# thomeou/SALSA

Measured on AMD Instinct MI355X. Metric: SALSA feat-extract audio-s/s, higher is better.
Workload: dtype f64 (STFT, noise-floor tracker, eigen-solve cold list) + packed f32 (covariance and eigen-solve of the certified frames); 1 GPU; Full SALSA FOA (eigenvector path): batch 32x60-s 4-ch 24 kHz clips per GPU, feature-extract only, n_fft 512 hop 300 fmax_doa 9000 cond 5 tracking on; clips_per_gpu=32, feature=salsa, format=foa, clip_groups=default

## Files before the change

salsa_amd/csrc/salsa_internal.h:

```cpp
#pragma once
#include <hip/hip_runtime.h>
#include <stdio.h>

#include "../../include/salsa_hip.h"
#include "salsa_math.h"

#define SALSA_LOCAL __attribute__((visibility("hidden")))

extern "C" SALSA_LOCAL void salsa_set_last_error_(const char *msg);

namespace salsa_impl {

static inline int fail(int code, const char *fmt, const char *a = "", long b = 0)
{
    char msg[512];
    snprintf(msg, sizeof(msg), fmt, a, b);
    salsa_set_last_error_(msg);
    return code;
}

static inline int hip_fail(const char *expr, hipError_t e)
{
    char msg[512];
    snprintf(msg, sizeof(msg), "%s failed: %s", expr, hipGetErrorString(e));
// ... 7 lines not shown
        if (e_ != hipSuccess) return salsa_impl::hip_fail(#expr, e_);                             \
    } while (0)

struct KParams {
    int B;
    int N;
    int T;
    int hop;
    int lower, upper, nd;
    int cutoff;
    int F;
    int OC;
    int ident;
    int spec_lo, spec_hi;
    int flex;
    int compress;
    int layout;
    int feature;
    int format;
    int tracking;
    int n_hop;
    int pair_sel;
    int nch;
    double cond;
    double inv_cond;
    double delta;
    double snr_ratio;
    const float *sc_mean;
    const float *sc_std;
    unsigned long long *stats;
    int force_f64;
    unsigned *doubt32;
    unsigned *doubt_flag;
};

constexpr int FEATURE_LOGSPEC_ONLY = 3;

constexpr int TR_CH = 64;
constexpr int TR_BINS = 32;
#ifndef K3_FT_N
#define K3_FT_N 8
#endif
constexpr int K3_FT = K3_FT_N;
#ifndef K3_NT_N
#define K3_NT_N 128
#endif
constexpr int K3_NT = K3_NT_N;
#ifndef SALSA_PK
#define SALSA_PK 1
#endif
#define SALSA_PK_COND_MIN 2.0

__device__ __forceinline__ int swz(int e) { return e ^ ((e >> 3) & 7); }

__device__ __forceinline__ void wave_lds_fence()
{
    __builtin_amdgcn_fence(__ATOMIC_RELEASE, "wavefront");
    __builtin_amdgcn_wave_barrier();
    __builtin_amdgcn_fence(__ATOMIC_ACQUIRE, "wavefront");
}

__device__ __forceinline__ float power32(const float2 x)
{
    const float t = x.x * x.x;
    return __builtin_fmaf(x.y, x.y, t);
}
// ... 69 lines not shown
```

salsa_amd/csrc/salsa_kernels.hip:

```cpp
#include "build_guard.h"
#include "salsa_internal.h"
#include <type_traits>

using salsa::cplx;
using namespace salsa_impl;

namespace {

template <int N> struct fft_cfg {
    static constexpr int NSUB = (N == 1024) ? 2 : 1;
    static constexpr int NS = N / NSUB;
    static constexpr int R = (NS == 512) ? 8 : 4;
    static constexpr int NP = (NS == 512) ? 2 : 3;
};

template <typename V> __device__ __forceinline__ V ld_off_c(const V *base, unsigned byte_off, int const_bytes) { return *(const V *)((const char *)base + byte_off + const_bytes); }
#ifndef K1_SPILL_NT
#define K1_SPILL_NT 1
#endif
typedef float salsa_f4v __attribute__((ext_vector_type(4)));
#ifndef TR_NT_LD
#define TR_NT_LD 0
#endif
#ifndef K3_GATHER_NT
// ... 449 lines not shown
        const double re = x[i].x, im = x[i].y;
        p[i] = re * re + im * im;
    }
#pragma unroll
    for (int i = 0; i < COUNT; i++) {
        if (first + i < TR_CH)
            dst[(first + i) * BINS + col] = raw ? sqrt(p[i + 2]) : sqrt(div3_exact(((0.0 + p[i + 2]) + p[i + 1]) + p[i]));
    }
}

#ifndef TR_IDLE4
#define TR_IDLE4 1
#endif
#ifndef TR_MASK_HISTORY
#define TR_MASK_HISTORY 1
#endif
#ifndef TR_CHUNK_CLAMP_SKIP
#define TR_CHUNK_CLAMP_SKIP 0
#endif
#ifndef TR_LAZY_CLAMP
#define TR_LAZY_CLAMP 0
#endif
extern "C" __device__ int salsa_writelane_i32(int value, int lane, int old) __asm("llvm.amdgcn.writelane.i32");
#ifndef TR_WIDE
#define TR_WIDE 0
#endif
constexpr int TR_WG_BINS = TR_WIDE ? 64 : TR_BINS;
static unsigned tracker_grid(const KParams &kp) { return (unsigned)(kp.B * ((kp.nd + TR_WG_BINS - 1) / TR_WG_BINS)); }

__global__ __launch_bounds__(64 * TR_WAVES) void tracker_kernel(const KParams kp, const float4 *__restrict__ Xs,
                                                                unsigned *__restrict__ valid32)
{
    if (kp.doubt_flag && blockIdx.x == 0 && threadIdx.x == 0) *kp.doubt_flag = 0u;
    constexpr int BINS = TR_WG_BINS, FS = 64 / BINS;
    constexpr bool IDLE4 = TR_WAVES > 4 && TR_IDLE4;
    constexpr int NPROD = IDLE4 ? TR_WAVES - 2 : TR_WAVES - 1;
    constexpr int PER_ALL = (TR_CH + TR_WAVES * FS - 1) / (TR_WAVES * FS);
    constexpr int PER_PROD = (TR_CH + NPROD * FS - 1) / (NPROD * FS);
    __shared__ double ring[2][TR_CH * BINS];
    const int ng32 = (kp.nd + BINS - 1) / BINS;
    const int b = blockIdx.x / ng32, g = blockIdx.x % ng32;
    const int w = __builtin_amdgcn_readfirstlane(threadIdx.x >> 6), lane = threadIdx.x & 63;
    const int col = lane % BINS, fsub = lane / BINS;
    const int bin = g * BINS + col;
    const bool active = bin < kp.nd;
    const int Tn = kp.T;
    const int stride = (kp.nch / 2) * kp.nd;
    const float4 *x0 = Xs + (long)b * Tn * stride + (active ? bin : 0);
    const int nchunks = (Tn + TR_CH - 1) / TR_CH;
    const bool raw = kp.flex != 0;
    {
        float2 x[PER_ALL + 2];
        const int first = (w * FS + fsub) * PER_ALL;
        tracker_load<PER_ALL>(kp, x0, stride, 0, first, active, x);
        tracker_mag<PER_ALL, BINS>(x, first, ring[0], col, raw);
    }
    float2 xa[PER_PROD + 2], xb[PER_PROD + 2];
    const bool producer = w > 0 && !(IDLE4 && w == 4);
    const int pidx = (IDLE4 && w > 4) ? w - 2 : w - 1;
    const int pfirst = (pidx * FS + fsub) * PER_PROD;
    if (producer && nchunks > 1) tracker_load<PER_PROD>(kp, x0, stride, TR_CH, pfirst, active, xa);
    __syncthreads();
    double fl = 0.0;
    int cd = 3;
    const double snr = kp.snr_ratio;
    const int n32 = (kp.nd + TR_BINS - 1) / TR_BINS;
// ... 119 lines not shown
#ifndef TR_PROBE_NO_PRODUCE
            if (w != 0 && producer) produce(c + 1, xb, xa);
#endif
        }
        chunk_barrier();
    }
}

#ifndef K3_GROUP
#define K3_GROUP 2
#endif
constexpr int K3_OW = K3_NT + 8;
#ifndef K3_XCD_CHUNK
#define K3_XCD_CHUNK 16
#endif

#ifndef K3_STAGE_LDS
#define K3_STAGE_LDS 0
#endif
#ifndef K3_OUT_NT
#define K3_OUT_NT 1
#endif
#ifndef K3_PK_WAVES
#define K3_PK_WAVES 4
#endif
template <bool FEAT, int NHOP, bool FAST = false, bool PK = false>
__global__ __launch_bounds__(K3_NT, PK ? K3_PK_WAVES : 1) void cov_eig_kernel(const KParams kp, const float4 *__restrict__ Xs,
                                                      const unsigned *__restrict__ valid32,
                                                      float *__restrict__ out_feat, double *__restrict__ out_eig,
                                                      unsigned char *__restrict__ gate)
{
    constexpr int G = NHOP >= 0 ? K3_GROUP : 1;
    constexpr bool PAIRED = G > 1;
    static_assert(K3_FT % G == 0 && G <= 4 && K3_FT / G <= 16, "work-list entry layout");
    __shared__ unsigned short list[K3_FT * K3_NT];
    __shared__ unsigned short slow[FAST ? K3_FT * K3_NT : 1];
    __shared__ int count, nslow;
    __shared__ __attribute__((aligned(16))) unsigned rowoff[NHOP >= 0 ? K3_FT + 2 * NHOP + 2 : 2];
    __shared__ __attribute__((aligned(16))) float otile[FEAT ? 3 * K3_FT * K3_OW : 4];
#if K3_STAGE_LDS
    __shared__ __attribute__((aligned(16))) float4 stage[PK ? (K3_FT + 6) * 2 * K3_NT : 1];
#endif
    const int tid = threadIdx.x;
    const int Tn = kp.T;
    int tile = blockIdx.x, b = blockIdx.y;
    if (K3_XCD_CHUNK > 0) {
        const unsigned ntile = gridDim.x, total = ntile * gridDim.y, lin = blockIdx.x + ntile * blockIdx.y;
        constexpr unsigned span = 8u * (K3_XCD_CHUNK > 0 ? K3_XCD_CHUNK : 1);
        if (lin < total / span * span) {
            const unsigned xcd = lin & 7u, j = lin >> 3;
            const unsigned tl = ((j / (span / 8)) * 8u + xcd) * (span / 8) + j % (span / 8);
            b = (int)(tl / ntile);
            tile = (int)(tl - (unsigned)b * ntile);
        }
    }
    const int t0 = tile * K3_FT;
    const int nft = Tn - t0 < K3_FT ? Tn - t0 : K3_FT;
    const int bin0 = blockIdx.z * K3_NT;
    const int nbc = kp.nd - bin0 < K3_NT ? kp.nd - bin0 : K3_NT;
    if (tid == 0) count = 0, nslow = 0;
    if (kp.doubt32 && tid < K3_FT * (K3_NT / 32)) {
        const int ft = tid % K3_FT, g32 = bin0 / 32 + tid / K3_FT, n32 = (kp.nd + TR_BINS - 1) / TR_BINS;
        if (ft < nft && g32 < n32) kp.doubt32[((long)b * n32 + g32) * Tn + t0 + ft] = 0u;
    }
    if (NHOP >= 0 && tid < K3_FT + 2 * NHOP) {
        int tt = t0 - NHOP + tid;
        while (tt < 0) tt += Tn;
        while (tt >= Tn) tt -= Tn;
        rowoff[tid] = (unsigned)tt * (16u * 2u * (unsigned)kp.nd);
    }
    if (FEAT) {
        for (int i = tid; i < 3 * K3_FT * K3_OW / 4; i += K3_NT) ((float4 *)otile)[i] = make_float4(0.f, 0.f, 0.f, 0.f);
    }
    __syncthreads();
    float *of = FEAT ? out_feat + ((long)b * kp.OC + 4) * Tn * kp.F : nullptr;
    double *oe = FEAT ? nullptr : out_eig + (long)b * 3 * kp.nd * Tn;
    unsigned char *og = (!FEAT && gate) ? gate + (long)b * kp.nd * Tn : nullptr;
    auto emit = [&](int t, int bin, const double *e, unsigned char g) {
        if (FEAT) {
#pragma unroll
            for (int i = 0; i < 3; i++) otile[(i * K3_FT + (t - t0)) * K3_OW + (bin - bin0)] = (float)e[i];
        } else {
#pragma unroll
            for (int i = 0; i < 3; i++) oe[((long)i * kp.nd + bin) * Tn + t] = e[i];
            if (og) og[(long)bin * Tn + t] = g;
        }
    };
    const double zero3[3] = {0.0, 0.0, 0.0};
    {
        const int bl = tid;
        const bool in = bl < nbc;
        const int ng32 = (kp.nd + TR_BINS - 1) / TR_BINS;
        const int bin = bin0 + bl;
        const int lane = tid & 63;
        const int grp = __builtin_amdgcn_readfirstlane(bin >> 6);
        const unsigned long long inmask = __ballot(in);
// ... 22 lines not shown
        int base = 0;
        if (lane == 0 && total) base = atomicAdd(&count, total);
        base = __builtin_amdgcn_readfirstlane(base);
#pragma unroll
        for (int ft = 0; ft < K3_FT; ft += G) {
            const unsigned long long wd = any_of(ft);
            if (in) {
                unsigned v = 0;
#pragma unroll
                for (int j = 0; j < G; j++) v |= ((unsigned)(words[ft + j] >> lane) & 1u) << j;
                if (v) list[base + __popcll(wd & ((1ull << lane) - 1))] = (unsigned short)((v << 12) | ((ft / G) << 8) | bl);
#pragma unroll
                for (int j = 0; j < G; j++)
                    if (!FEAT && ft + j < nft && !((v >> j) & 1)) emit(t0 + ft + j, bin, zero3, 0);
            }
            base += __popcll(wd);
        }
    }
    const int seg = (FEAT && blockIdx.z == gridDim.z - 1) ? (kp.F - bin0 < K3_OW ? kp.F - bin0 : K3_OW) : nbc;
    if (FEAT && blockIdx.z == gridDim.z - 1 && kp.F - bin0 > K3_OW) {
        const int first = bin0 + K3_OW, tail = kp.F - first;
        for (int i = tid; i < nft * tail; i += K3_NT) {
            const int ft = i / tail, f = first + (i - ft * tail);
#pragma unroll
            for (int c = 0; c < 3; c++) st_off(of, 4u * (unsigned)((c * Tn + t0 + ft) * kp.F + f), 0.f);
        }
    }
    __syncthreads();
    const int n = count;
    const int stride = 2 * kp.nd;
    const int nhop = NHOP >= 0 ? NHOP : kp.n_hop;
    const float4 *xclip = Xs + (long)b * Tn * stride;
    const bool ungated = !kp.tracking && !kp.flex;
    auto solve_emit = [&](const salsa::herm4<double> &R, int t, int bin, auto path) {
        constexpr int PATH = decltype(path)::value;
        const bool foa = kp.format == SALSA_FORMAT_FOA;
        const salsa::eig_result<double> er = salsa::herm4_gate_eigvec<PATH>(R, kp.cond, kp.inv_cond, ungated, !foa);
        if (PATH == 1 && er.fallback) {
            slow[atomicAdd(&nslow, 1)] = (unsigned short)(((t - t0) << 8) | (bin - bin0));
            return;
        }
        if (er.doubt && kp.doubt32 && !ungated) {
            atomicOr(&kp.doubt32[((long)b * ((kp.nd + TR_BINS - 1) / TR_BINS) + (bin >> 5)) * Tn + t], 1u << (bin & 31));
            atomicOr(kp.doubt_flag, 1u);
        }
        double e[3] = {0.0, 0.0, 0.0};
        unsigned char g = er.rank1 ? 2 : 1;
        if (er.rank1 || ungated) {
            const int k = bin + kp.lower;
            const double den = kp.flex ? (double)((float)(k == 0 ? 1 : k) * (float)kp.delta) : kp.delta * (double)k;
            if (PATH != 2 && er.col0) {
                if (foa) salsa::normalise_foa_col0(er.u, e);
                else salsa::normalise_mic_col0(er.u, den, e);
            } else if (PATH != 1) {
                if (foa) salsa::normalise_foa(er.u, e, ungated);
                else salsa::normalise_mic(er.u, den, e);
            }
            g = 2;
        } else if (FEAT && kp.flex && !kp.tracking) {
            e[0] = __builtin_nan("");
        }
        emit(t, bin, e, g);
    };
    using hot_path = std::integral_constant<int, FAST ? 1 : 2>;
    using cold_path = std::integral_constant<int, 2>;
    if constexpr (PK) {
        static_assert(!PK || (G == 2 && FEAT && FAST && NHOP >= 0), "the packed solve takes the two frames of a pair");
        constexpr int NW = 2 * NHOP + 2;
        const unsigned half = 16u * (unsigned)kp.nd;
#if K3_STAGE_LDS
        if (n > 0) {
            for (int i = tid; i < (K3_FT + 6) * 2 * K3_NT; i += K3_NT) {
// ... 26 lines not shown
            auto chans = [&](int k, salsa::pk2f *v) {
                v[0] = salsa::pk2f{xa[k].x, xa[k].y};
                v[1] = salsa::pk2f{xa[k].z, xa[k].w};
                v[2] = salsa::pk2f{xc[k].x, xc[k].y};
                v[3] = salsa::pk2f{xc[k].z, xc[k].w};
            };
            salsa::cov4pk Cc = {}, C0, C1;
            salsa::pk2f v[4];
#pragma unroll
            for (int k = 1; k <= 2 * NHOP; k++) {
                chans(k, v);
                salsa::cov4pk_rank1(Cc, Cc, v);
            }
            chans(0, v);
            salsa::cov4pk_rank1(C0, Cc, v);
            chans(2 * NHOP + 1, v);
            salsa::cov4pk_rank1(C1, Cc, v);
            const int live = (i >> 12) & 3;
            int odd;
            const salsa::herm4<salsa::pk2f> A = salsa::herm4_pk_from_windows(C0, C1, odd);
            salsa::pk2f e[3];
            salsa::pk_eig r;
            if (kp.format == SALSA_FORMAT_FOA) {
                r = salsa::herm4_gate_eigvec_pk<false>(A, (float)kp.cond, (float)kp.inv_cond, live & ~odd);
                if (r.pass) salsa::normalise_foa_pk(r, e);
            } else {
                r = salsa::herm4_gate_eigvec_pk<true>(A, (float)kp.cond, (float)kp.inv_cond, live & ~odd);
                if (r.pass) salsa::normalise_mic_pk(r, (float)(kp.delta * (double)(bin0 + bl + kp.lower)), e);
            }
            r.unsure |= odd & live;
#pragma unroll
            for (int j = 0; j < 2; j++) {
                if ((r.unsure >> j) & 1)
                    slow[atomicAdd(&nslow, 1)] = (unsigned short)(((ft + j) << 8) | bl);
                else if ((r.pass >> j) & 1) {
#pragma unroll
                    for (int q = 0; q < 3; q++) otile[(q * K3_FT + ft + j) * K3_OW + bl] = e[q][j];
                }
            }
        }
    }
    for (int s = tid; !PK && s < n; s += K3_NT) {
        const int i = list[s];
        const int t = t0 + G * ((i >> 8) & 15);
        const int bin = bin0 + (i & 255);
        const float4 *xb = xclip + bin;
        const unsigned row = 16u * (unsigned)stride, boff = 16u * (unsigned)bin, half = 16u * (unsigned)kp.nd;
        if (PAIRED) {
            constexpr int NW = NHOP >= 0 ? 2 * NHOP + G : G;
            float4 xa[NW], xc[NW];
            const unsigned *ro = rowoff + (t - t0);
#pragma unroll
            for (int k = 0; k < NW; k++) {
                const unsigned r = ro[k];
                xa[k] = ld_off(xclip, r + boff);
                xc[k] = ld_off(xclip, r + boff + half);
            }
            auto frame = [&](int k, salsa::herm4<double> &A) {
                const cplx<double> x[4] = {{(double)xa[k].x, (double)xa[k].y}, {(double)xa[k].z, (double)xa[k].w},
                                           {(double)xc[k].x, (double)xc[k].y}, {(double)xc[k].z, (double)xc[k].w}};
                salsa::herm4_rank1_add(A, x);
            };
            salsa::herm4<double> Rc = {};
#pragma unroll
            for (int k = G - 1; k <= 2 * NHOP; k++) frame(k, Rc);
#pragma unroll
            for (int j = 0; j < G; j++) {
                if ((i >> (12 + j)) & 1) {
                    salsa::herm4<double> R = Rc;
#pragma unroll
                    for (int k = j; k < G - 1; k++) frame(k, R);
#pragma unroll
                    for (int k = 2 * NHOP + 1; k <= 2 * NHOP + j; k++) frame(k, R);
                    solve_emit(R, t + j, bin, hot_path{});
                }
            }
        } else {
            salsa::herm4<double> R = {};
            for (int k = -nhop; k <= nhop; k++) {
                int tt = t + k;
                while (tt < 0) tt += Tn;
                while (tt >= Tn) tt -= Tn;
                const float4 a = xb[tt * stride], c = xb[tt * stride + kp.nd];
                const cplx<double> x[4] = {{(double)a.x, (double)a.y}, {(double)a.z, (double)a.w},
                                           {(double)c.x, (double)c.y}, {(double)c.z, (double)c.w}};
                salsa::herm4_rank1_add(R, x);
            }
            solve_emit(R, t, bin, hot_path{});
        }
    }
    if (FAST) {
        __syncthreads();
        const int ns = nslow;
        if (kp.stats && tid == 0) {
            int live = 0;
            for (int s = 0; s < n; s++) live += __popc((list[s] >> 12) & 15);
            atomicAdd(&kp.stats[0], (unsigned long long)n);
            atomicAdd(&kp.stats[1], (unsigned long long)live);
            atomicAdd(&kp.stats[2], (unsigned long long)ns);
            atomicAdd(&kp.stats[3], 1ull);
        }
        for (int s = tid; s < ns; s += K3_NT) {
            const int i = slow[s];
            const int t = t0 + (i >> 8), bin = bin0 + (i & 255);
            const float4 *xb = xclip + bin;
            salsa::herm4<double> R = {};
            for (int k = -nhop; k <= nhop; k++) {
                int tt = t + k;
                while (tt < 0) tt += Tn;
                while (tt >= Tn) tt -= Tn;
                const float4 a = xb[tt * stride], c = xb[tt * stride + kp.nd];
                const cplx<double> x[4] = {{(double)a.x, (double)a.y}, {(double)a.z, (double)a.w},
                                           {(double)c.x, (double)c.y}, {(double)c.z, (double)c.w}};
                salsa::herm4_rank1_add(R, x);
            }
            solve_emit(R, t, bin, cold_path{});
        }
    }
    if (FEAT) {
        __syncthreads();
        const bool vec = !(kp.F & 3) && !(seg & 3) && !(bin0 & 3);
        if (vec) {
            const int q = seg >> 2;
            for (int i = tid; i < 3 * nft * q; i += K3_NT) {
                const int row = i / q, col = i - row * q, c = row / nft, ft = row - c * nft;
                float4 *dst = (float4 *)(of + ((long)(c * Tn + t0 + ft) * kp.F + bin0 + 4 * col));
                const float4 val = *(const float4 *)(otile + (c * K3_FT + ft) * K3_OW + 4 * col);
                if (K3_OUT_NT) st_off_nt(dst, 0u, val);
                else *dst = val;
            }
        } else {
            for (int i = tid; i < 3 * nft * seg; i += K3_NT) {
                const int row = i / seg, col = i - row * seg, c = row / nft, ft = row - c * nft;
                of[(long)(c * Tn + t0 + ft) * kp.F + bin0 + col] = otile[(c * K3_FT + ft) * K3_OW + col];
            }
        }
    }
}

template <bool FEAT>
__global__ __launch_bounds__(256) void gate_doubt_kernel(const KParams kp, const float4 *__restrict__ Xs, float *__restrict__ out_feat,
                                                         double *__restrict__ out_eig, unsigned char *__restrict__ gate)
{
    if (*(const volatile unsigned *)kp.doubt_flag == 0u) return;
    const int Tn = kp.T, n32 = (kp.nd + TR_BINS - 1) / TR_BINS, stride = 2 * kp.nd;
    const long nwords = (long)kp.B * n32 * Tn;
    const bool foa = kp.format == SALSA_FORMAT_FOA;
    for (long wi = (long)blockIdx.x * blockDim.x + threadIdx.x; wi < nwords; wi += (long)gridDim.x * blockDim.x) {
        unsigned word = kp.doubt32[wi];
        if (!word) continue;
        const int t = (int)(wi % Tn), g32 = (int)((wi / Tn) % n32), b = (int)(wi / ((long)Tn * n32));
        while (word) {
            const int j = __ffs((int)word) - 1;
            word &= word - 1u;
            const int bin = 32 * g32 + j;
            const float4 *xb = Xs + (long)b * Tn * stride + bin;
            salsa::herm4<double> R = {};
            for (int k = -kp.n_hop; k <= kp.n_hop; k++) {
                int tt = t + k;
                while (tt < 0) tt += Tn;
                while (tt >= Tn) tt -= Tn;
                const float4 a = xb[tt * stride], c = xb[tt * stride + kp.nd];
                const cplx<double> x[4] = {{(double)a.x, (double)a.y}, {(double)a.z, (double)a.w},
                                           {(double)c.x, (double)c.y}, {(double)c.z, (double)c.w}};
                salsa::herm4_rank1_add(R, x);
            }
            const bool rank1 = salsa::herm4_rank1_by_jacobi(R, kp.cond);
            double e[3] = {0.0, 0.0, 0.0};
            if (rank1) {
                const salsa::eig_result<double> er = salsa::herm4_gate_eigvec<2>(R, kp.cond, kp.inv_cond, true, !foa);
                const int k = bin + kp.lower;
                const double den = kp.flex ? (double)((float)(k == 0 ? 1 : k) * (float)kp.delta) : kp.delta * (double)k;
                if (foa) salsa::normalise_foa(er.u, e, false);
                else salsa::normalise_mic(er.u, den, e);
            } else if (FEAT && kp.flex && !kp.tracking) {
                e[0] = __builtin_nan("");
            }
            if (FEAT) {
#pragma unroll
                for (int i = 0; i < 3; i++) out_feat[(((long)b * kp.OC + 4 + i) * Tn + t) * kp.F + bin] = (float)e[i];
            } else {
#pragma unroll
                for (int i = 0; i < 3; i++) out_eig[(((long)b * 3 + i) * kp.nd + bin) * Tn + t] = e[i];
                if (gate) gate[((long)b * kp.nd + bin) * Tn + t] = rank1 ? 2 : 1;
            }
        }
    }
}

__global__ __launch_bounds__(256) void flex_allpass_kernel(const KParams kp, float *__restrict__ out)
{
    const int bin = blockIdx.x * 256 + threadIdx.x;
    if (bin >= kp.nd) return;
    float *of = out + ((long)blockIdx.y * kp.OC + kp.nch) * kp.T * kp.F + bin;
    bool dead = false;
    for (int t = 0; t < kp.T; t++) {
        const float v = of[t * kp.F];
        dead = dead || (v != v);
        if (dead) {
            for (int c = 0; c < kp.nch - 1; c++) of[(c * kp.T + t) * kp.F] = 0.f;
        }
    }
}

}

namespace salsa_impl {

void launch_tracker(const KParams &kp, hipStream_t s, const float4 *Xs, unsigned *valid32)
{
    hipLaunchKernelGGL(tracker_kernel, dim3(tracker_grid(kp)), dim3(64 * TR_WAVES), 0, s, kp, Xs, valid32);
}

template <bool FEAT>
static void launch_gate_doubt(const KParams &kp, hipStream_t s, const float4 *Xs, float *out_feat, double *out_eig, unsigned char *gate)
{
    if (!kp.doubt32) return;
    const long nwords = (long)kp.B * ((kp.nd + TR_BINS - 1) / TR_BINS) * kp.T;
    const unsigned blocks = (unsigned)(nwords < 256L * 64 ? (nwords + 255) / 256 : 64);
    hipLaunchKernelGGL(gate_doubt_kernel<FEAT>, dim3(blocks ? blocks : 1u), dim3(256), 0, s, kp, Xs, out_feat, out_eig, gate);
}

template <bool FEAT>
void launch_cov_eig(const KParams &kp, dim3 grid, hipStream_t s, const float4 *Xs, const unsigned *valid,
                    float *out_feat, double *out_eig, unsigned char *gate)
{
    const bool gated = kp.tracking || kp.flex;
    if (kp.doubt32 && !kp.tracking) (void)hipMemsetAsync(kp.doubt_flag, 0, sizeof(unsigned), s);
    if (FEAT && SALSA_PK && K3_GROUP == 2 && kp.n_hop == 3 && gated && SALSA_COL0 && !kp.flex && kp.cond >= SALSA_PK_COND_MIN && kp.cond < 1e6 && !kp.force_f64)
        hipLaunchKernelGGL((cov_eig_kernel<FEAT, 3, true, FEAT && K3_GROUP == 2>), grid, dim3(K3_NT), 0, s, kp, Xs, valid, out_feat, out_eig, gate);
    else if (kp.n_hop == 3 && gated && SALSA_COL0)
        hipLaunchKernelGGL((cov_eig_kernel<FEAT, 3, true>), grid, dim3(K3_NT), 0, s, kp, Xs, valid, out_feat, out_eig, gate);
    else if (kp.n_hop == 3)
        hipLaunchKernelGGL((cov_eig_kernel<FEAT, 3>), grid, dim3(K3_NT), 0, s, kp, Xs, valid, out_feat, out_eig, gate);
    else
        hipLaunchKernelGGL((cov_eig_kernel<FEAT, -1>), grid, dim3(K3_NT), 0, s, kp, Xs, valid, out_feat, out_eig, gate);
    launch_gate_doubt<FEAT>(kp, s, Xs, out_feat, out_eig, gate);
}

template void launch_cov_eig<true>(const KParams &, dim3, hipStream_t, const float4 *, const unsigned *, float *, double *, unsigned char *);
template void launch_cov_eig<false>(const KParams &, dim3, hipStream_t, const float4 *, const unsigned *, float *, double *, unsigned char *);

void launch_flex_allpass(const KParams &kp, hipStream_t s, float *out)
{
    hipLaunchKernelGGL(flex_allpass_kernel, dim3((unsigned)((kp.nd + 255) / 256), (unsigned)kp.B), dim3(256), 0, s, kp, out);
}

int launch_stft(salsa_plan *pl, const KParams &kp, const double *win, const float *d_audio, float *d_out, float4 *Xs, hipStream_t s)
{
    const bool lite = kp.feature == SALSA_FEATURE_LITE || kp.feature == SALSA_FEATURE_IPD;
    const bool single = !lite && kp.pair_sel >= 0;
    constexpr int NF_FULL = k1_cfg<false>::NF, NF_LITE = k1_cfg<true>::NF, NF_PAIR = 2 * k1_cfg<false>::NF;
    const int fpb = 4 * (lite ? NF_LITE : single ? NF_PAIR : NF_FULL);
    const unsigned nblk = (unsigned)((kp.T + fpb - 1) / fpb);
    dim3 grid(nblk, (unsigned)kp.B);
    const bool one_window = pl->d_window == pl->d_window_doa;
    const bool std_layout = K1_STD && one_window && pl->p.n_fft == 512 && !lite && !single && kp.feature == SALSA_FEATURE_SALSA && kp.compress &&
                            kp.spec_lo == 1 && kp.spec_hi == 193 && kp.ident == 192 && kp.F == 200 && kp.nch == 4 &&
                            kp.layout == SALSA_LAYOUT_PLANAR && kp.pair_sel < 0;
    const bool lite_std = K1_LITE_STD && one_window && pl->p.n_fft == 512 && lite && kp.nch == 4 && kp.layout == SALSA_LAYOUT_PLANAR && !kp.sc_mean &&
                          kp.cutoff <= 256 && kp.pair_sel < 0;
    if (lite_std) {
        hipLaunchKernelGGL((stft_kernel<512, double, true, NF_LITE, 2, false, true>), grid, dim3(256), 0, s, kp, d_audio, win, pl->d_tw, d_out, Xs);
    } else if (std_layout) {
        constexpr size_t SCT_BYTES = 2 * 4 * 256 * sizeof(float);
        if (kp.sc_mean) hipLaunchKernelGGL((stft_kernel<512, double, false, NF_FULL, 2, true, true>), grid, dim3(256), SCT_BYTES, s, kp, d_audio, win, pl->d_tw, d_out, Xs);
        else hipLaunchKernelGGL((stft_kernel<512, double, false, NF_FULL, 2, false, true>), grid, dim3(256), 0, s, kp, d_audio, win, pl->d_tw, d_out, Xs);
    } else if (pl->p.n_fft == 1024) {
        if (!lite) return fail(SALSA_ENFFT, "n_fft 1024 is a SALSA-Lite / SALSA-IPD size%s");
        hipLaunchKernelGGL((stft_kernel<1024, double, true, NF_LITE>), grid, dim3(256), 0, s, kp, d_audio, win, pl->d_tw, d_out, Xs);
// ... 49 lines not shown
```

salsa_amd/csrc/salsa_plan.hip:

```cpp
#include "build_guard.h"
#include "salsa_internal.h"
#include <string.h>

using salsa::cplx;
using namespace salsa_impl;

namespace {

thread_local char g_err[512] = "";

}

namespace salsa_impl {

KParams make_kparams(const salsa_plan *pl, int batch, int64_t n_samples)
{
    KParams kp;
    memset(&kp, 0, sizeof(kp));
    kp.B = batch;
    kp.N = (int)n_samples;
    kp.T = (int)(1 + n_samples / pl->p.hop_len);
    kp.hop = pl->p.hop_len;
    kp.lower = pl->lower;
    kp.upper = pl->upper;
// ... 184 lines not shown

int salsa_plan_destroy(salsa_plan *pl)
{
    if (!pl) return SALSA_OK;
    if (pl->d_window) (void)hipFree(pl->d_window);
    if (pl->d_tw) (void)hipFree(pl->d_tw);
    for (int i = 0; i < SALSA_MAX_KERNELS; i++) {
        if (pl->ev0[i]) (void)hipEventDestroy(pl->ev0[i]);
        if (pl->ev1[i]) (void)hipEventDestroy(pl->ev1[i]);
    }
    for (int i = 0; i <= SALSA_MAX_GROUPS; i++) {
        if (pl->streams[i]) (void)hipStreamDestroy(pl->streams[i]);
        if (pl->ev_join[i]) (void)hipEventDestroy(pl->ev_join[i]);
        if (i < SALSA_MAX_GROUPS && pl->ev_stft[i]) (void)hipEventDestroy(pl->ev_stft[i]);
        if (i < SALSA_MAX_GROUPS && pl->ev_stft2[i]) (void)hipEventDestroy(pl->ev_stft2[i]);
    }
    if (pl->gexec) (void)hipGraphExecDestroy(pl->gexec);
    if (pl->cap_stream) (void)hipStreamDestroy(pl->cap_stream);
    if (pl->ev_fork) (void)hipEventDestroy(pl->ev_fork);
    delete pl;
    return SALSA_OK;
}

int salsa_output_shape(const salsa_plan *pl, int64_t n_samples, int *C, int64_t *T, int *F)
{
    if (!pl || n_samples < 0) return fail(SALSA_EINVAL, "salsa_output_shape: bad argument%s");
    if (C) *C = 7;
    if (T) *T = 1 + n_samples / pl->p.hop_len;
    if (F) *F = pl->F;
    return SALSA_OK;
}

static size_t mask_bytes(int batch, size_t T, int nd) { return align256((size_t)batch * ((T + 63) / 64) * ((nd + 63) / 64) * 64 * 8); }

size_t salsa_workspace_bytes(const salsa_plan *pl, int batch, int64_t n_samples)
{
    if (!pl || batch <= 0 || n_samples <= 0 || pl->p.feature_type != SALSA_FEATURE_SALSA) return 0;
    const size_t T = 1 + n_samples / pl->p.hop_len;
    return align256((size_t)batch * T * 4 * pl->nd * sizeof(float2)) + 2 * mask_bytes(batch, T, pl->nd) + align256(sizeof(unsigned) * (size_t)batch) + 256;
}

size_t salsa_eigvec_workspace_bytes(const salsa_plan *pl, int batch, int n_bins, int64_t n_frames)
{
    if (!pl || batch <= 0 || n_bins <= 0 || n_frames <= 0) return 0;
    return align256((size_t)batch * n_frames * 4 * n_bins * sizeof(float2)) + 2 * mask_bytes(batch, (size_t)n_frames, n_bins) + align256(sizeof(unsigned) * (size_t)batch) + 256;
}

static int mark_begin(salsa_plan *pl, hipStream_t s, const char *name)
{
    if (!pl->timing || pl->n_kernels >= SALSA_MAX_KERNELS) return -1;
    const int i = pl->n_kernels++;
    pl->names[i] = name;
    if (!pl->ev0[i]) (void)hipEventCreate(&pl->ev0[i]);
    if (!pl->ev1[i]) (void)hipEventCreate(&pl->ev1[i]);
    (void)hipEventRecord(pl->ev0[i], s);
    return i;
}
static void mark_end(salsa_plan *pl, hipStream_t s, int i)
{
    if (i >= 0) (void)hipEventRecord(pl->ev1[i], s);
}

int salsa_extract_batch(salsa_plan *pl, const float *d_audio, int batch, int64_t n_samples, float *d_out,
                        void *d_workspace, size_t workspace_bytes, void *hip_stream)
{
    if (!pl || !d_audio || !d_out || batch <= 0 || n_samples <= 0)
        return fail(SALSA_EINVAL, "salsa_extract_batch: bad argument%s");
    if (n_samples <= pl->p.n_fft / 2)
        return fail(SALSA_EINVAL, "clip shorter than n_fft/2 samples cannot be reflect-padded%s");
    {
        int cur = -1;
        if (hipGetDevice(&cur) != hipSuccess || cur != pl->device)
            return fail(SALSA_EINVAL, "the plan's tables live on the device that was current at salsa_plan_create; make it current%s");
    }
    {
        const int64_t T64 = 1 + n_samples / pl->p.hop_len;
        if (n_samples * 16 >= INT32_MAX || T64 * 7 * pl->F >= INT32_MAX / 2 || T64 * 2 * (pl->nd > 0 ? pl->nd : 1) >= INT32_MAX / 8)
            return fail(SALSA_EINVAL, "clip too long for 32-bit per-clip indexing (split it)%s");
        if ((T64 + K3_FT - 1) / K3_FT > 65535) return fail(SALSA_EINVAL, "clip too long for one launch (split it)%s");
    }
    hipStream_t s = (hipStream_t)hip_stream;
    KParams kp = make_kparams(pl, batch, n_samples);
    const bool full = pl->p.feature_type == SALSA_FEATURE_SALSA;
    float4 *Xs = nullptr;
    unsigned *valid = nullptr;
    if (full) {
        const size_t need = salsa_workspace_bytes(pl, batch, n_samples);
        if (!d_workspace || workspace_bytes < need) return fail(SALSA_EWORKSPACE, "workspace too small%s (need %ld bytes)", "", (long)need);
        Xs = (float4 *)d_workspace;
        valid = (unsigned *)((unsigned char *)d_workspace + align256((size_t)batch * kp.T * 4 * kp.nd * sizeof(float2)));
        if ((kp.tracking || kp.flex) && kp.cond > 1.0 && kp.nd > 0) {
            kp.doubt32 = (unsigned *)((unsigned char *)valid + mask_bytes(batch, (size_t)kp.T, kp.nd));
            kp.doubt_flag = (unsigned *)((unsigned char *)kp.doubt32 + mask_bytes(batch, (size_t)kp.T, kp.nd));
        }
    }
    pl->n_kernels = 0;
    const long T = kp.T;
    const size_t nchunks = (size_t)((T + TR_CH - 1) / TR_CH);
    auto run_group = [&](int g0, int g1, hipStream_t s1, hipStream_t s2, hipEvent_t after_first, hipEvent_t after_second,
                         bool split) -> int {
        KParams gp = kp;
        gp.B = g1 - g0;
        const float *a = d_audio + (size_t)g0 * 4 * kp.N;
        float *o = d_out + (size_t)g0 * 7 * T * kp.F;
        float4 *xs = Xs ? Xs + (size_t)g0 * T * 2 * kp.nd : nullptr;
        unsigned *vm = valid ? valid + (size_t)g0 * ((kp.nd + TR_BINS - 1) / TR_BINS) * T : nullptr;
        if (kp.doubt32) gp.doubt32 = kp.doubt32 + (size_t)g0 * ((kp.nd + TR_BINS - 1) / TR_BINS) * T, gp.doubt_flag = kp.doubt_flag + g0;
        const bool two = split && full && gp.nd > 0;
        gp.pair_sel = two ? 0 : -1;
        const int reps = pl->timing > 1 ? pl->timing : 1;
        int m = mark_begin(pl, s1, "stft_logspec");
        int rc = SALSA_OK;
        for (int r = 0; r < reps && !rc; r++) rc = launch_k1(pl, gp, a, o, xs, s1);
        mark_end(pl, s1, m);
        if (rc || !full) return rc;
        if (pl->stop_after == 1) return SALSA_PARTIAL;
        if (s1 != s2) {
            HIP_TRY(hipEventRecord(after_first, s1));
            HIP_TRY(hipStreamWaitEvent(s2, after_first, 0));
        }
        if (gp.nd == 0) {
            HIP_TRY(hipMemset2DAsync(o + 4 * T * kp.F, sizeof(float) * 7 * T * kp.F, 0, sizeof(float) * 3 * T * kp.F, (size_t)gp.B, s2));
            return SALSA_OK;
        }
        if (two) {
            gp.pair_sel = 1;
            m = mark_begin(pl, s1, "stft_logspec");
            rc = launch_stft(pl, gp, pl->d_window, a, o, xs, s1);
            mark_end(pl, s1, m);
            if (rc) return rc;
            gp.pair_sel = -1;
            if (s1 != s2) HIP_TRY(hipEventRecord(after_second, s1));
        }
        if (gp.tracking) {
            m = mark_begin(pl, s2, "noise_floor_tracker");
            for (int r = 0; r < reps; r++) launch_tracker(gp, s2, xs, vm);
            mark_end(pl, s2, m);
            HIP_TRY(hipGetLastError());
        }
        if (pl->stop_after == 2) return SALSA_PARTIAL;
// ... 87 lines not shown
        return fail(SALSA_EINVAL, "clip too long for 32-bit per-clip indexing (split it)%s");
    KParams kp = make_kparams(pl, batch, n_samples);
    kp.feature = FEATURE_LOGSPEC_ONLY;
    kp.OC = 4;
    kp.sc_mean = kp.sc_std = nullptr;
    kp.layout = SALSA_LAYOUT_PLANAR;
    kp.F = freq_dim(pl->p.n_fft, pl->p.is_compress_high_freq);
    kp.ident = pl->p.is_compress_high_freq ? (pl->p.n_fft == 512 ? 192 : 96) : pl->p.n_fft / 2;
    kp.compress = pl->p.is_compress_high_freq;
    kp.spec_lo = 1;
    kp.spec_hi = kp.ident + 1;
    return launch_stft(pl, kp, pl->d_window, d_audio, d_out, nullptr, (hipStream_t)hip_stream);
}

int salsa_eigvec_batch(salsa_plan *pl, const float *d_X, int batch, int n_bins, int64_t n_frames, int lower_bin,
                       double *d_out, unsigned char *d_gate, void *d_workspace, size_t workspace_bytes,
                       void *hip_stream)
{
    if (!pl || !d_X || !d_out || batch <= 0 || n_bins <= 0 || n_frames <= 0)
        return fail(SALSA_EINVAL, "salsa_eigvec_batch: bad argument%s");
    if ((int64_t)n_frames * 2 * n_bins >= INT32_MAX) return fail(SALSA_EINVAL, "block too large for 32-bit per-clip indexing%s");
    const size_t need = salsa_eigvec_workspace_bytes(pl, batch, n_bins, n_frames);
    if (!d_workspace || workspace_bytes < need) return fail(SALSA_EWORKSPACE, "workspace too small%s (need %ld bytes)", "", (long)need);
    hipStream_t s = (hipStream_t)hip_stream;
    KParams kp = make_kparams(pl, batch, 0);
    kp.T = (int)n_frames;
    kp.nd = n_bins;
    kp.lower = lower_bin;
    kp.upper = lower_bin + n_bins;
    kp.F = n_bins;
    kp.feature = SALSA_FEATURE_SALSA;
    float4 *Xs = (float4 *)d_workspace;
    unsigned *valid = (unsigned *)((unsigned char *)d_workspace + align256((size_t)batch * n_frames * 4 * n_bins * sizeof(float2)));
    if ((kp.tracking || kp.flex) && kp.cond > 1.0) {
        kp.doubt32 = (unsigned *)((unsigned char *)valid + mask_bytes(batch, (size_t)n_frames, n_bins));
        kp.doubt_flag = (unsigned *)((unsigned char *)kp.doubt32 + mask_bytes(batch, (size_t)n_frames, n_bins));
    }
    launch_relayout((const float4 *)d_X, Xs, batch, n_bins, (int)n_frames, s);
    HIP_TRY(hipGetLastError());
    if (kp.tracking) {
        launch_tracker(kp, s, Xs, valid);
        HIP_TRY(hipGetLastError());
    }
    const unsigned ntile = (unsigned)((kp.T + K3_FT - 1) / K3_FT);
    dim3 grid(ntile, (unsigned)kp.B, (unsigned)((n_bins + K3_NT - 1) / K3_NT));
    launch_cov_eig<false>(kp, grid, s, Xs, valid, (float *)nullptr, d_out, d_gate);
    HIP_TRY(hipGetLastError());
    return SALSA_OK;
}

int salsa_eigvec_feature_batch(salsa_plan *pl, const float *d_X, int batch, int n_bins, int64_t n_frames, int lower_bin,
                               float *d_feat, void *d_workspace, size_t workspace_bytes, void *hip_stream)
{
    if (!pl || !d_X || !d_feat || batch <= 0 || n_bins <= 0 || n_frames <= 0)
        return fail(SALSA_EINVAL, "salsa_eigvec_feature_batch: bad argument%s");
    if ((int64_t)n_frames * 2 * n_bins >= INT32_MAX / 8 || (int64_t)n_frames * 7 * n_bins >= INT32_MAX / 2)
        return fail(SALSA_EINVAL, "block too large for 32-bit per-clip indexing%s");
    if ((n_frames + K3_FT - 1) / K3_FT > 65535) return fail(SALSA_EINVAL, "block too long for one launch%s");
    const size_t need = salsa_eigvec_workspace_bytes(pl, batch, n_bins, n_frames);
    if (!d_workspace || workspace_bytes < need) return fail(SALSA_EWORKSPACE, "workspace too small%s (need %ld bytes)", "", (long)need);
    hipStream_t s = (hipStream_t)hip_stream;
    KParams kp = make_kparams(pl, batch, 0);
    kp.T = (int)n_frames;
    kp.nd = n_bins;
    kp.lower = lower_bin;
    kp.upper = lower_bin + n_bins;
    kp.F = n_bins;
    kp.OC = 7;
    kp.feature = SALSA_FEATURE_SALSA;
    float4 *Xs = (float4 *)d_workspace;
    unsigned *valid = (unsigned *)((unsigned char *)d_workspace + align256((size_t)batch * n_frames * 4 * n_bins * sizeof(float2)));
    if ((kp.tracking || kp.flex) && kp.cond > 1.0) {
        kp.doubt32 = (unsigned *)((unsigned char *)valid + mask_bytes(batch, (size_t)n_frames, n_bins));
        kp.doubt_flag = (unsigned *)((unsigned char *)kp.doubt32 + mask_bytes(batch, (size_t)n_frames, n_bins));
    }
    launch_relayout((const float4 *)d_X, Xs, batch, n_bins, (int)n_frames, s);
    HIP_TRY(hipGetLastError());
    if (kp.tracking) {
        launch_tracker(kp, s, Xs, valid);
        HIP_TRY(hipGetLastError());
    }
    const unsigned ntile = (unsigned)((kp.T + K3_FT - 1) / K3_FT);
    dim3 grid(ntile, (unsigned)kp.B, (unsigned)((n_bins + K3_NT - 1) / K3_NT));
    launch_cov_eig<true>(kp, grid, s, Xs, valid, d_feat, (double *)nullptr, (unsigned char *)nullptr);
    HIP_TRY(hipGetLastError());
    return SALSA_OK;
}

int salsa_plan_set_fused(salsa_plan *pl, int mode)
{
    if (!pl || mode < 0 || mode > 2) return fail(SALSA_EINVAL, "salsa_plan_set_fused: bad argument%s");
    pl->fused = mode;
    return SALSA_OK;
}

int salsa_plan_set_stats(salsa_plan *pl, unsigned long long *d_counters)
{
    if (!pl) return fail(SALSA_EINVAL, "salsa_plan_set_stats: NULL plan%s");
    pl->stats = d_counters;
    return SALSA_OK;
}

int salsa_plan_set_timing(salsa_plan *pl, int enable)
{
    if (!pl) return fail(SALSA_EINVAL, "salsa_plan_set_timing: NULL plan%s");
    pl->timing = enable > 0 ? enable : 0;
    pl->stop_after = enable < 0 ? (enable >= -2 ? -enable : 0) : 0;
    pl->n_kernels = 0;
// ... 64 lines not shown
```

Measured before the change: 1.981 million audio-seconds/s.

## Defer cold-path f64 eigen-solves to a separate compacted kernel via bitmask

In the packed fast FEAT path, frames that fail the f32 certification are no longer solved in f64 inside the same cov_eig block. Instead each one sets a bit in a new global cold32 mask. A merged cold/doubt kernel later compacts those bits into an LDS list and solves them across the whole grid. This removes the load imbalance and serial tail in each tile where a few threads did slow f64 solves while the rest sat idle, and it frees the slow LDS array. The cost is global atomics, an extra mask, more workspace, and a second pass that recomputes the covariances from memory.

```diff
diff --git a/salsa_amd/csrc/salsa_internal.h b/salsa_amd/csrc/salsa_internal.h
--- a/salsa_amd/csrc/salsa_internal.h
+++ b/salsa_amd/csrc/salsa_internal.h
@@ -63,6 +63,8 @@
     int force_f64;
     unsigned *doubt32;
     unsigned *doubt_flag;
+    unsigned *cold32;
+    unsigned *cold_flag;
 };
 
 constexpr int FEATURE_LOGSPEC_ONLY = 3;
diff --git a/salsa_amd/csrc/salsa_kernels.hip b/salsa_amd/csrc/salsa_kernels.hip
--- a/salsa_amd/csrc/salsa_kernels.hip
+++ b/salsa_amd/csrc/salsa_kernels.hip
@@ -505,6 +505,7 @@
                                                                 unsigned *__restrict__ valid32)
 {
     if (kp.doubt_flag && blockIdx.x == 0 && threadIdx.x == 0) *kp.doubt_flag = 0u;
+    if (kp.cold_flag && blockIdx.x == 0 && threadIdx.x == 0) *kp.cold_flag = 0u;
     constexpr int BINS = TR_WG_BINS, FS = 64 / BINS;
     constexpr bool IDLE4 = TR_WAVES > 4 && TR_IDLE4;
     constexpr int NPROD = IDLE4 ? TR_WAVES - 2 : TR_WAVES - 1;
@@ -690,9 +691,10 @@
 {
     constexpr int G = NHOP >= 0 ? K3_GROUP : 1;
     constexpr bool PAIRED = G > 1;
+    constexpr bool DEFER = FAST && FEAT;
     static_assert(K3_FT % G == 0 && G <= 4 && K3_FT / G <= 16, "work-list entry layout");
     __shared__ unsigned short list[K3_FT * K3_NT];
-    __shared__ unsigned short slow[FAST ? K3_FT * K3_NT : 1];
+    __shared__ unsigned short slow[FAST && !DEFER ? K3_FT * K3_NT : 1];
     __shared__ int count, nslow;
     __shared__ __attribute__((aligned(16))) unsigned rowoff[NHOP >= 0 ? K3_FT + 2 * NHOP + 2 : 2];
     __shared__ __attribute__((aligned(16))) float otile[FEAT ? 3 * K3_FT * K3_OW : 4];
@@ -720,6 +722,10 @@
     if (kp.doubt32 && tid < K3_FT * (K3_NT / 32)) {
         const int ft = tid % K3_FT, g32 = bin0 / 32 + tid / K3_FT, n32 = (kp.nd + TR_BINS - 1) / TR_BINS;
         if (ft < nft && g32 < n32) kp.doubt32[((long)b * n32 + g32) * Tn + t0 + ft] = 0u;
+    }
+    if (DEFER && tid < K3_FT * (K3_NT / 32)) {
+        const int ft = tid % K3_FT, g32 = bin0 / 32 + tid / K3_FT, n32 = (kp.nd + TR_BINS - 1) / TR_BINS;
+        if (ft < nft && g32 < n32) kp.cold32[((long)b * n32 + g32) * Tn + t0 + ft] = 0u;
     }
     if (NHOP >= 0 && tid < K3_FT + 2 * NHOP) {
         int tt = t0 - NHOP + tid;
@@ -808,12 +814,21 @@
     const int nhop = NHOP >= 0 ? NHOP : kp.n_hop;
     const float4 *xclip = Xs + (long)b * Tn * stride;
     const bool ungated = !kp.tracking && !kp.flex;
+    auto push_cold = [&](int ft, int bl) {
+        if constexpr (DEFER) {
+            const int bin = bin0 + bl;
+            atomicOr(&kp.cold32[((long)b * ((kp.nd + TR_BINS - 1) / TR_BINS) + (bin >> 5)) * Tn + t0 + ft], 1u << (bin & 31));
+            atomicAdd(&nslow, 1);
+        } else {
+            slow[atomicAdd(&nslow, 1)] = (unsigned short)((ft << 8) | bl);
+        }
+    };
     auto solve_emit = [&](const salsa::herm4<double> &R, int t, int bin, auto path) {
         constexpr int PATH = decltype(path)::value;
         const bool foa = kp.format == SALSA_FORMAT_FOA;
         const salsa::eig_result<double> er = salsa::herm4_gate_eigvec<PATH>(R, kp.cond, kp.inv_cond, ungated, !foa);
         if (PATH == 1 && er.fallback) {
-            slow[atomicAdd(&nslow, 1)] = (unsigned short)(((t - t0) << 8) | (bin - bin0));
+            push_cold(t - t0, bin - bin0);
             return;
         }
         if (er.doubt && kp.doubt32 && !ungated) {
@@ -906,7 +921,7 @@
 #pragma unroll
             for (int j = 0; j < 2; j++) {
                 if ((r.unsure >> j) & 1)
-                    slow[atomicAdd(&nslow, 1)] = (unsigned short)(((ft + j) << 8) | bl);
+                    push_cold(ft + j, bl);
                 else if ((r.pass >> j) & 1) {
 #pragma unroll
                     for (int q = 0; q < 3; q++) otile[(q * K3_FT + ft + j) * K3_OW + bl] = e[q][j];
@@ -963,9 +978,7 @@
             solve_emit(R, t, bin, hot_path{});
         }
     }
-    if (FAST) {
-        __syncthreads();
-        const int ns = nslow;
+    auto count_stats = [&](int ns) {
         if (kp.stats && tid == 0) {
             int live = 0;
             for (int s = 0; s < n; s++) live += __popc((list[s] >> 12) & 15);
@@ -974,6 +987,11 @@
             atomicAdd(&kp.stats[2], (unsigned long long)ns);
             atomicAdd(&kp.stats[3], 1ull);
         }
+    };
+    if constexpr (FAST && !DEFER) {
+        __syncthreads();
+        const int ns = nslow;
+        count_stats(ns);
         for (int s = tid; s < ns; s += K3_NT) {
             const int i = slow[s];
             const int t = t0 + (i >> 8), bin = bin0 + (i & 255);
@@ -993,6 +1011,11 @@
     }
     if (FEAT) {
         __syncthreads();
+        if constexpr (DEFER) {
+            const int ns = nslow;
+            count_stats(ns);
+            if (tid == 0 && ns && *(const volatile unsigned *)kp.cold_flag == 0u) atomicOr(kp.cold_flag, 1u);
+        }
         const bool vec = !(kp.F & 3) && !(seg & 3) && !(bin0 & 3);
         if (vec) {
             const int q = seg >> 2;
@@ -1012,14 +1035,130 @@
     }
 }
 
+constexpr int CD_NT = 256;
+constexpr int CD_ROUNDS = 4;
+constexpr int CD_GRAN = 8;
+constexpr int CD_CAP = CD_NT - 1 + 32 * CD_NT;
+
+template <int NHOP = -1>
+__device__ __forceinline__ void cold_covariance(const KParams &kp, const float4 *xb, int t, salsa::herm4<double> &R)
+{
+    const int Tn = kp.T, stride = 2 * kp.nd;
+    auto wrapped = [&](int tt) {
+        while (tt < 0) tt += Tn;
+        while (tt >= Tn) tt -= Tn;
+        return tt;
+    };
+    auto add = [&](const float4 a, const float4 c) {
+        const cplx<double> x[4] = {{(double)a.x, (double)a.y}, {(double)a.z, (double)a.w},
+                                   {(double)c.x, (double)c.y}, {(double)c.z, (double)c.w}};
+        salsa::herm4_rank1_add(R, x);
+    };
+    if constexpr (NHOP >= 0) {
+        float4 xa[2 * NHOP + 1], xc[2 * NHOP + 1];
+#pragma unroll
+        for (int k = 0; k <= 2 * NHOP; k++) {
+            const int tt = wrapped(t + k - NHOP);
+            xa[k] = xb[tt * stride], xc[k] = xb[tt * stride + kp.nd];
+        }
+#pragma unroll
+        for (int k = 0; k <= 2 * NHOP; k++) add(xa[k], xc[k]);
+    } else {
+        for (int k = -kp.n_hop; k <= kp.n_hop; k++) {
+            const int tt = wrapped(t + k);
+            add(xb[tt * stride], xb[tt * stride + kp.nd]);
+        }
+    }
+}
+
 template <bool FEAT>
-__global__ __launch_bounds__(256) void gate_doubt_kernel(const KParams kp, const float4 *__restrict__ Xs, float *__restrict__ out_feat,
-                                                         double *__restrict__ out_eig, unsigned char *__restrict__ gate)
-{
-    if (*(const volatile unsigned *)kp.doubt_flag == 0u) return;
+__device__ __forceinline__ bool doubt_decide(const KParams &kp, const salsa::herm4<double> &R, int bin, double *e)
+{
+    const bool foa = kp.format == SALSA_FORMAT_FOA;
+    const bool rank1 = salsa::herm4_rank1_by_jacobi(R, kp.cond);
+    e[0] = e[1] = e[2] = 0.0;
+    if (rank1) {
+        const salsa::eig_result<double> er = salsa::herm4_gate_eigvec<2>(R, kp.cond, kp.inv_cond, true, !foa);
+        const int k = bin + kp.lower;
+        const double den = kp.flex ? (double)((float)(k == 0 ? 1 : k) * (float)kp.delta) : kp.delta * (double)k;
+        if (foa) salsa::normalise_foa(er.u, e, false);
+        else salsa::normalise_mic(er.u, den, e);
+    } else if (FEAT && kp.flex && !kp.tracking) {
+        e[0] = __builtin_nan("");
+    }
+    return rank1;
+}
+
+template <bool FEAT>
+__global__ __launch_bounds__(CD_NT) void cold_doubt_kernel(const KParams kp, const float4 *__restrict__ Xs, float *__restrict__ out_feat,
+                                                           double *__restrict__ out_eig, unsigned char *__restrict__ gate)
+{
+    const bool any_cold = FEAT && kp.cold32 && *(const volatile unsigned *)kp.cold_flag != 0u;
+    const bool any_doubt = kp.doubt32 && *(const volatile unsigned *)kp.doubt_flag != 0u;
+    if (!any_cold && !any_doubt) return;
     const int Tn = kp.T, n32 = (kp.nd + TR_BINS - 1) / TR_BINS, stride = 2 * kp.nd;
     const long nwords = (long)kp.B * n32 * Tn;
     const bool foa = kp.format == SALSA_FORMAT_FOA;
+    if constexpr (FEAT) {
+        __shared__ unsigned clist[CD_CAP];
+        __shared__ int cn;
+        const int tid = threadIdx.x;
+        if (any_cold) {
+            const long ngran = (nwords + CD_GRAN - 1) / CD_GRAN;
+            auto word_of = [&](long g0, int slot) { return ((g0 + slot / CD_GRAN) * gridDim.x + blockIdx.x) * CD_GRAN + slot % CD_GRAN; };
+            for (long g0 = 0; g0 * gridDim.x < ngran; g0 += CD_ROUNDS * (CD_NT / CD_GRAN)) {
+                unsigned w[CD_ROUNDS];
+#pragma unroll
+                for (int r = 0; r < CD_ROUNDS; r++) {
+                    const long wi = word_of(g0, r * CD_NT + tid);
+                    w[r] = wi < nwords ? kp.cold32[wi] : 0u;
+                }
+                if (tid == 0) cn = 0;
+                __syncthreads();
+#pragma unroll
+                for (int r = 0; r < CD_ROUNDS; r++) {
+                    unsigned word = w[r];
+                    if (word) {
+                        int at = atomicAdd(&cn, __popc(word));
+                        while (word) {
+                            clist[at++] = ((unsigned)(r * CD_NT + tid) << 5) | (unsigned)(__ffs((int)word) - 1);
+                            word &= word - 1u;
+                        }
+                    }
+                    __syncthreads();
+                    const int n = cn;
+                    __syncthreads();
+                    if (n < CD_NT && r + 1 < CD_ROUNDS) continue;
+                    for (int s = tid; s < n; s += CD_NT) {
+                        const unsigned ent = clist[s];
+                        const long wi = word_of(g0, (int)(ent >> 5));
+                        const int t = (int)(wi % Tn), g32 = (int)((wi / Tn) % n32), b = (int)(wi / ((long)Tn * n32));
+                        const int bin = 32 * g32 + (int)(ent & 31u);
+                        salsa::herm4<double> R = {};
+                        cold_covariance<3>(kp, Xs + (long)b * Tn * stride + bin, t, R);
+                        const salsa::eig_result<double> er = salsa::herm4_gate_eigvec<2>(R, kp.cond, kp.inv_cond, false, !foa);
+                        double e[3] = {0.0, 0.0, 0.0};
+                        if (er.doubt && kp.doubt32) {
+                            doubt_decide<FEAT>(kp, R, bin, e);
+                        } else if (er.rank1) {
+                            const int k = bin + kp.lower;
+                            const double den = kp.flex ? (double)((float)(k == 0 ? 1 : k) * (float)kp.delta) : kp.delta * (double)k;
+                            if (foa) salsa::normalise_foa(er.u, e, false);
+                            else salsa::normalise_mic(er.u, den, e);
+                        } else if (kp.flex && !kp.tracking) {
+                            e[0] = __builtin_nan("");
+                        }
+#pragma unroll
+                        for (int i = 0; i < 3; i++) out_feat[(((long)b * kp.OC + 4 + i) * Tn + t) * kp.F + bin] = (float)e[i];
+                    }
+                    __syncthreads();
+                    if (tid == 0) cn = 0;
+                    __syncthreads();
+                }
+            }
+        }
+    }
+    if (!any_doubt) return;
     for (long wi = (long)blockIdx.x * blockDim.x + threadIdx.x; wi < nwords; wi += (long)gridDim.x * blockDim.x) {
         unsigned word = kp.doubt32[wi];
         if (!word) continue;
@@ -1028,28 +1167,10 @@
             const int j = __ffs((int)word) - 1;
             word &= word - 1u;
             const int bin = 32 * g32 + j;
-            const float4 *xb = Xs + (long)b * Tn * stride + bin;
             salsa::herm4<double> R = {};
-            for (int k = -kp.n_hop; k <= kp.n_hop; k++) {
-                int tt = t + k;
-                while (tt < 0) tt += Tn;
-                while (tt >= Tn) tt -= Tn;
-                const float4 a = xb[tt * stride], c = xb[tt * stride + kp.nd];
-                const cplx<double> x[4] = {{(double)a.x, (double)a.y}, {(double)a.z, (double)a.w},
-                                           {(double)c.x, (double)c.y}, {(double)c.z, (double)c.w}};
-                salsa::herm4_rank1_add(R, x);
-            }
-            const bool rank1 = salsa::herm4_rank1_by_jacobi(R, kp.cond);
-            double e[3] = {0.0, 0.0, 0.0};
-            if (rank1) {
-                const salsa::eig_result<double> er = salsa::herm4_gate_eigvec<2>(R, kp.cond, kp.inv_cond, true, !foa);
-                const int k = bin + kp.lower;
-                const double den = kp.flex ? (double)((float)(k == 0 ? 1 : k) * (float)kp.delta) : kp.delta * (double)k;
-                if (foa) salsa::normalise_foa(er.u, e, false);
-                else salsa::normalise_mic(er.u, den, e);
-            } else if (FEAT && kp.flex && !kp.tracking) {
-                e[0] = __builtin_nan("");
-            }
+            cold_covariance(kp, Xs + (long)b * Tn * stride + bin, t, R);
+            double e[3];
+            const bool rank1 = doubt_decide<FEAT>(kp, R, bin, e);
             if (FEAT) {
 #pragma unroll
                 for (int i = 0; i < 3; i++) out_feat[(((long)b * kp.OC + 4 + i) * Tn + t) * kp.F + bin] = (float)e[i];
@@ -1087,12 +1208,15 @@
 }
 
 template <bool FEAT>
-static void launch_gate_doubt(const KParams &kp, hipStream_t s, const float4 *Xs, float *out_feat, double *out_eig, unsigned char *gate)
-{
-    if (!kp.doubt32) return;
+static void launch_cold_doubt(KParams kp, bool cold, hipStream_t s, const float4 *Xs, float *out_feat, double *out_eig, unsigned char *gate)
+{
+    if (!cold) kp.cold32 = nullptr, kp.cold_flag = nullptr;
+    if (!kp.doubt32 && !kp.cold32) return;
     const long nwords = (long)kp.B * ((kp.nd + TR_BINS - 1) / TR_BINS) * kp.T;
-    const unsigned blocks = (unsigned)(nwords < 256L * 64 ? (nwords + 255) / 256 : 64);
-    hipLaunchKernelGGL(gate_doubt_kernel<FEAT>, dim3(blocks ? blocks : 1u), dim3(256), 0, s, kp, Xs, out_feat, out_eig, gate);
+    long blocks = nwords < 256L * 64 ? (nwords + 255) / 256 : 64;
+    if (kp.cold32) blocks = (nwords + (long)CD_ROUNDS * CD_NT - 1) / ((long)CD_ROUNDS * CD_NT);
+    if (blocks > 65535) blocks = 65535;
+    hipLaunchKernelGGL(cold_doubt_kernel<FEAT>, dim3((unsigned)(blocks ? blocks : 1)), dim3(CD_NT), 0, s, kp, Xs, out_feat, out_eig, gate);
 }
 
 template <bool FEAT>
@@ -1101,6 +1225,8 @@
 {
     const bool gated = kp.tracking || kp.flex;
     if (kp.doubt32 && !kp.tracking) (void)hipMemsetAsync(kp.doubt_flag, 0, sizeof(unsigned), s);
+    if (kp.cold32 && !kp.tracking) (void)hipMemsetAsync(kp.cold_flag, 0, sizeof(unsigned), s);
+    const bool fast = kp.n_hop == 3 && gated && SALSA_COL0;
     if (FEAT && SALSA_PK && K3_GROUP == 2 && kp.n_hop == 3 && gated && SALSA_COL0 && !kp.flex && kp.cond >= SALSA_PK_COND_MIN && kp.cond < 1e6 && !kp.force_f64)
         hipLaunchKernelGGL((cov_eig_kernel<FEAT, 3, true, FEAT && K3_GROUP == 2>), grid, dim3(K3_NT), 0, s, kp, Xs, valid, out_feat, out_eig, gate);
     else if (kp.n_hop == 3 && gated && SALSA_COL0)
@@ -1109,7 +1235,7 @@
         hipLaunchKernelGGL((cov_eig_kernel<FEAT, 3>), grid, dim3(K3_NT), 0, s, kp, Xs, valid, out_feat, out_eig, gate);
     else
         hipLaunchKernelGGL((cov_eig_kernel<FEAT, -1>), grid, dim3(K3_NT), 0, s, kp, Xs, valid, out_feat, out_eig, gate);
-    launch_gate_doubt<FEAT>(kp, s, Xs, out_feat, out_eig, gate);
+    launch_cold_doubt<FEAT>(kp, FEAT && fast && kp.cold32, s, Xs, out_feat, out_eig, gate);
 }
 
 template void launch_cov_eig<true>(const KParams &, dim3, hipStream_t, const float4 *, const unsigned *, float *, double *, unsigned char *);
diff --git a/salsa_amd/csrc/salsa_plan.hip b/salsa_amd/csrc/salsa_plan.hip
--- a/salsa_amd/csrc/salsa_plan.hip
+++ b/salsa_amd/csrc/salsa_plan.hip
@@ -240,18 +240,31 @@
 }
 
 static size_t mask_bytes(int batch, size_t T, int nd) { return align256((size_t)batch * ((T + 63) / 64) * ((nd + 63) / 64) * 64 * 8); }
+static size_t flag_bytes(int batch) { return align256(sizeof(unsigned) * (size_t)batch); }
+
+static void place_gate_masks(KParams &kp, unsigned *valid, int batch, size_t T, int nd)
+{
+    unsigned char *p = (unsigned char *)valid + mask_bytes(batch, T, nd);
+    if (kp.cond > 1.0) {
+        kp.doubt32 = (unsigned *)p;
+        kp.doubt_flag = (unsigned *)(p + mask_bytes(batch, T, nd));
+    }
+    p += mask_bytes(batch, T, nd) + flag_bytes(batch);
+    kp.cold32 = (unsigned *)p;
+    kp.cold_flag = (unsigned *)(p + mask_bytes(batch, T, nd));
+}
 
 size_t salsa_workspace_bytes(const salsa_plan *pl, int batch, int64_t n_samples)
 {
     if (!pl || batch <= 0 || n_samples <= 0 || pl->p.feature_type != SALSA_FEATURE_SALSA) return 0;
     const size_t T = 1 + n_samples / pl->p.hop_len;
-    return align256((size_t)batch * T * 4 * pl->nd * sizeof(float2)) + 2 * mask_bytes(batch, T, pl->nd) + align256(sizeof(unsigned) * (size_t)batch) + 256;
+    return align256((size_t)batch * T * 4 * pl->nd * sizeof(float2)) + 3 * mask_bytes(batch, T, pl->nd) + 2 * flag_bytes(batch) + 256;
 }
 
 size_t salsa_eigvec_workspace_bytes(const salsa_plan *pl, int batch, int n_bins, int64_t n_frames)
 {
     if (!pl || batch <= 0 || n_bins <= 0 || n_frames <= 0) return 0;
-    return align256((size_t)batch * n_frames * 4 * n_bins * sizeof(float2)) + 2 * mask_bytes(batch, (size_t)n_frames, n_bins) + align256(sizeof(unsigned) * (size_t)batch) + 256;
+    return align256((size_t)batch * n_frames * 4 * n_bins * sizeof(float2)) + 3 * mask_bytes(batch, (size_t)n_frames, n_bins) + 2 * flag_bytes(batch) + 256;
 }
 
 static int mark_begin(salsa_plan *pl, hipStream_t s, const char *name)
@@ -297,10 +310,7 @@
         if (!d_workspace || workspace_bytes < need) return fail(SALSA_EWORKSPACE, "workspace too small%s (need %ld bytes)", "", (long)need);
         Xs = (float4 *)d_workspace;
         valid = (unsigned *)((unsigned char *)d_workspace + align256((size_t)batch * kp.T * 4 * kp.nd * sizeof(float2)));
-        if ((kp.tracking || kp.flex) && kp.cond > 1.0 && kp.nd > 0) {
-            kp.doubt32 = (unsigned *)((unsigned char *)valid + mask_bytes(batch, (size_t)kp.T, kp.nd));
-            kp.doubt_flag = (unsigned *)((unsigned char *)kp.doubt32 + mask_bytes(batch, (size_t)kp.T, kp.nd));
-        }
+        if ((kp.tracking || kp.flex) && kp.nd > 0) place_gate_masks(kp, valid, batch, (size_t)kp.T, kp.nd);
     }
     pl->n_kernels = 0;
     const long T = kp.T;
@@ -314,6 +324,7 @@
         float4 *xs = Xs ? Xs + (size_t)g0 * T * 2 * kp.nd : nullptr;
         unsigned *vm = valid ? valid + (size_t)g0 * ((kp.nd + TR_BINS - 1) / TR_BINS) * T : nullptr;
         if (kp.doubt32) gp.doubt32 = kp.doubt32 + (size_t)g0 * ((kp.nd + TR_BINS - 1) / TR_BINS) * T, gp.doubt_flag = kp.doubt_flag + g0;
+        if (kp.cold32) gp.cold32 = kp.cold32 + (size_t)g0 * ((kp.nd + TR_BINS - 1) / TR_BINS) * T, gp.cold_flag = kp.cold_flag + g0;
         const bool two = split && full && gp.nd > 0;
         gp.pair_sel = two ? 0 : -1;
         const int reps = pl->timing > 1 ? pl->timing : 1;
@@ -467,10 +478,7 @@
     kp.feature = SALSA_FEATURE_SALSA;
     float4 *Xs = (float4 *)d_workspace;
     unsigned *valid = (unsigned *)((unsigned char *)d_workspace + align256((size_t)batch * n_frames * 4 * n_bins * sizeof(float2)));
-    if ((kp.tracking || kp.flex) && kp.cond > 1.0) {
-        kp.doubt32 = (unsigned *)((unsigned char *)valid + mask_bytes(batch, (size_t)n_frames, n_bins));
-        kp.doubt_flag = (unsigned *)((unsigned char *)kp.doubt32 + mask_bytes(batch, (size_t)n_frames, n_bins));
-    }
+    if (kp.tracking || kp.flex) place_gate_masks(kp, valid, batch, (size_t)n_frames, n_bins);
     launch_relayout((const float4 *)d_X, Xs, batch, n_bins, (int)n_frames, s);
     HIP_TRY(hipGetLastError());
     if (kp.tracking) {
@@ -505,10 +513,7 @@
     kp.feature = SALSA_FEATURE_SALSA;
     float4 *Xs = (float4 *)d_workspace;
     unsigned *valid = (unsigned *)((unsigned char *)d_workspace + align256((size_t)batch * n_frames * 4 * n_bins * sizeof(float2)));
-    if ((kp.tracking || kp.flex) && kp.cond > 1.0) {
-        kp.doubt32 = (unsigned *)((unsigned char *)valid + mask_bytes(batch, (size_t)n_frames, n_bins));
-        kp.doubt_flag = (unsigned *)((unsigned char *)kp.doubt32 + mask_bytes(batch, (size_t)n_frames, n_bins));
-    }
+    if (kp.tracking || kp.flex) place_gate_masks(kp, valid, batch, (size_t)n_frames, n_bins);
     launch_relayout((const float4 *)d_X, Xs, batch, n_bins, (int)n_frames, s);
     HIP_TRY(hipGetLastError());
     if (kp.tracking) {
```

New measurement: 1.986 million audio-seconds/s (median of 2 runs). About the same (+0.2%).
